# voithru/voice-activity-detection

Hardware: AMD Instinct MI355X
Metric: audio frames/sec (whole node) (higher is better)
Workload: dtype f32 (bf16x6 split operands, f32 accumulate)

## Files before the change

### voice_activity_detection_amd/csrc/savad.hip

```cpp
#include "savad_kernels.h"
#include "savad_kernels_bf16.h"
#include "savad_attn_pw_bf16.h"
#include "savad_packed_bf16.h"
#include "savad_kernels_f32s.h"
#include "savad_generic.h"
#include <type_traits>
#include "savad_logmel.h"
#include "savad_frontend.h"
#include "savad_ingest.h"
#include "savad_post.h"

#include <math.h>
#include <stdarg.h>
#include <stdio.h>
#include <string.h>

#include <map>
#include <mutex>
#include <string>
#include <vector>

#include "../../include/savad.h"

#define SAVAD_EXPORT extern "C" __attribute__((visibility("default")))
// ... 27 lines not shown
constexpr int MAX_EVENTS = 64;

}

struct savad_model {
    savad_config cfg;
    bool generic = false;
    std::vector<Param> params;
    float* d_raw = nullptr;
    float* d_packed = nullptr;
    size_t raw_floats = 0, packed_floats = 0;
    bool dirty = true;
    float* d_pe = nullptr;
    int pe_len = 0;
    std::vector<float> h_pe;
    int splits = 0;
    int row_mode = 0;
    bool batch_invariant = false;
    int precision = 0;
    char* d_frag3 = nullptr;
    size_t frag3_bytes = 0;
    bool frag3_dirty = true;
    bool lds_attrs3_set = false;
    size_t f3_win = 0;
    unsigned* d_sat = nullptr;
    char* d_frag = nullptr;
    size_t frag_bytes = 0;
    bool frag_dirty = true;
    bool lds_attrs_set = false;
    int n_cu = 256;
    size_t f_win = 0;
    struct LayerFrag {
        size_t wqkv, wo, w1, w2;
    };
    std::vector<LayerFrag> lf;
    std::vector<LayerFrag> lf3;
    int prof_capacity = 0, prof_used = 0, prof_nk = 0, prof_skip = 0;
    std::vector<hipEvent_t> events;
    std::vector<const char*> knames;

    size_t r_win, r_bin, r_lnf_w, r_lnf_b, r_wc, r_bc;
    struct LayerRaw {
        size_t wq, bq, wk, bk, wv, bv, wo, bo, ln1w, ln1b, w1, b1, w2, b2, ln2w, ln2b;
    };
    std::vector<LayerRaw> lr;
    struct LayerPacked {
        size_t wqkv, bqkv, w1, b1;
        size_t frag;
    };
    std::vector<LayerPacked> lp;
    size_t p_wc, p_bc;
    size_t p_bias = 0;
    int FP = 0;
    size_t p_win_pad = 0;
};

namespace {

using namespace savad;

size_t add_param(savad_model* m, const std::string& key, size_t numel) {
    const size_t off = m->raw_floats;
    m->params.push_back(Param{key, numel, off, false});
    m->raw_floats += (numel + 3) & ~size_t(3);
    return off;
}

int choose_splits(const savad_model* m, int B, int T) {
    if (T <= 32) return 1;
    const int NT = (T + 31) / 32, QB = NT;
    if (m->splits > 0) return m->splits < NT ? m->splits : NT;
    auto cost = [&](int S) {
        const long wgs = (long)B * ((QB + 3) / 4) * S;
        return (double)((wgs + 255) / 256) * ((NT + S - 1) / S + 1.5);
    };
    const double cost1 = cost(1);
    double best = cost1;
    int bestS = 1;
    for (int S = 2; S <= 8 && S <= NT; ++S) {
        const double cs = cost(S);
// ... 238 lines not shown
#define SAVAD_F32S_PACKED_MIN_BLOCKS 0
#endif
bool packed_f32s_applies(const savad_model* m, int B, int T) {
    if (T > 32 || m->cfg.num_layers > fs::PACKED_F32S_MAX_LAYERS) return false;
    const long nblk = ((long)B + 32 / T - 1) / (32 / T);
    return m->row_mode >= 4 || (m->row_mode == 0 && nblk >= SAVAD_F32S_PACKED_MIN_BLOCKS);
}
#ifndef SAVAD_F32S_MIN_BLOCKS_PER_CU
#define SAVAD_F32S_MIN_BLOCKS_PER_CU 1
#endif
bool f32s_uses_exact_fp32(const savad_model* m, int B, int T) {
    if (m->row_mode != 0) return false;
    if (T <= 32) return !packed_f32s_applies(m, B, T);
    return (long)B * ((T + 31) / 32) <= (long)SAVAD_F32S_MIN_BLOCKS_PER_CU * m->n_cu;
}
int pack_frags3(savad_model* m, hipStream_t st, const float* W, int N, int K, size_t off) {
    const size_t total = (size_t)N * K;
    const int grid = (int)((total + 255) / 256 < 1024 ? (total + 255) / 256 : 1024);
    hipLaunchKernelGGL(fs::pack_weight_frags3_kernel, dim3(grid), dim3(256), 0, st, W, N, K, reinterpret_cast<__bf16*>(m->d_frag3 + off));
    HIP_TRY(hipGetLastError());
    return SAVAD_OK;
}

int prepare_frags3(savad_model* m, hipStream_t st) {
    if (!m->frag3_dirty) return SAVAD_OK;
    const int L = m->cfg.num_layers;
    int rc;
    if ((rc = pack_frags3(m, st, win_fp32(m), D, m->FP, m->f3_win))) return rc;
    for (int l = 0; l < L; ++l) {
        if ((rc = pack_frags3(m, st, m->d_packed + m->lp[l].wqkv, 3 * D, D, m->lf3[l].wqkv))) return rc;
        if ((rc = pack_frags3(m, st, m->d_raw + m->lr[l].wo, D, D, m->lf3[l].wo))) return rc;
        if ((rc = pack_frags3(m, st, m->d_packed + m->lp[l].w1, DFF, D, m->lf3[l].w1))) return rc;
        if ((rc = pack_frags3(m, st, m->d_raw + m->lr[l].w2, D, DFF, m->lf3[l].w2))) return rc;
    }
    m->frag3_dirty = false;
    return SAVAD_OK;
}

template <typename KernelT>
int allow_lds(KernelT kernel, int bytes) {
    HIP_TRY(hipFuncSetAttribute(reinterpret_cast<const void*>(kernel), hipFuncAttributeMaxDynamicSharedMemorySize, bytes));
    return SAVAD_OK;
}

struct Prof {
    savad_model* m;
    hipStream_t st;
    hipEvent_t* ev;
    int n;
    Prof(savad_model* mm, hipStream_t s) : m(mm), st(s), ev(nullptr), n(0) {
        if (m->prof_capacity > 0 && m->prof_skip > 0) {
            --m->prof_skip;
        } else if (m->prof_capacity > 0 && m->prof_used < m->prof_capacity) {
            ev = m->events.data() + (size_t)m->prof_used * MAX_EVENTS;
            m->knames.clear();
            hipEventRecord(ev[0], st);
        }
    }
    void mark(const char* name) {
        if (!ev || n + 1 >= MAX_EVENTS) return;
        ++n;
        hipEventRecord(ev[n], st);
        m->knames.push_back(name);
    }
    void done() {
        if (!ev) return;
// ... 181 lines not shown
    const int F = cfg->feature_size, L = cfg->num_layers;
    m->r_win = add_param(m, "input_layer.0.weight", (size_t)D * F);
    m->r_bin = add_param(m, "input_layer.0.bias", D);
    m->lr.resize(L);
    m->lp.resize(L);
    for (int l = 0; l < L; ++l) {
        const std::string p = "encoder.layers." + std::to_string(l) + ".";
        auto& r = m->lr[l];
        r.wq = add_param(m, p + "self_attention.query_projection.weight", (size_t)D * D);
        r.bq = add_param(m, p + "self_attention.query_projection.bias", D);
        r.wk = add_param(m, p + "self_attention.key_projection.weight", (size_t)D * D);
        r.bk = add_param(m, p + "self_attention.key_projection.bias", D);
        r.wv = add_param(m, p + "self_attention.value_projection.weight", (size_t)D * D);
        r.bv = add_param(m, p + "self_attention.value_projection.bias", D);
        r.wo = add_param(m, p + "self_attention.final_projection.weight", (size_t)D * D);
        r.bo = add_param(m, p + "self_attention.final_projection.bias", D);
        r.ln1w = add_param(m, p + "self_attention_sublayer.layer_norm.weight", D);
        r.ln1b = add_param(m, p + "self_attention_sublayer.layer_norm.bias", D);
        r.w1 = add_param(m, p + "feed_forward.feed_forward.0.weight", (size_t)DFF * D);
        r.b1 = add_param(m, p + "feed_forward.feed_forward.0.bias", DFF);
        r.w2 = add_param(m, p + "feed_forward.feed_forward.3.weight", (size_t)D * DFF);
        r.b2 = add_param(m, p + "feed_forward.feed_forward.3.bias", D);
        r.ln2w = add_param(m, p + "feed_forward_sublayer.layer_norm.weight", D);
        r.ln2b = add_param(m, p + "feed_forward_sublayer.layer_norm.bias", D);
        auto& q = m->lp[l];
        q.wqkv = m->packed_floats;
        m->packed_floats += (size_t)3 * D * D;
        q.bqkv = m->packed_floats;
        m->packed_floats += 3 * D;
        q.w1 = m->packed_floats;
        m->packed_floats += (size_t)DFF * D;
        q.b1 = m->packed_floats;
        m->packed_floats += DFF;
        q.frag = m->packed_floats;
        m->packed_floats += FRAG_LAYER;
    }
    m->r_lnf_w = add_param(m, "encoder.layer_norm.weight", D);
    m->r_lnf_b = add_param(m, "encoder.layer_norm.bias", D);
    m->r_wc = add_param(m, "classifier.weight", 2 * D);
    m->r_bc = add_param(m, "classifier.bias", 2);
    m->p_bias = m->packed_floats;
    m->packed_floats += (size_t)L * LBIAS;
    m->p_wc = m->packed_floats;
    m->packed_floats += 2 * D;
    m->p_bc = m->packed_floats;
    m->packed_floats += 4;
    m->FP = (F + 15) / 16 * 16;
    m->p_win_pad = m->packed_floats;
    m->packed_floats += (size_t)D * m->FP;
    m->lf.resize(L);
    m->f_win = 0;
    m->frag_bytes = (size_t)D * ((F + 15) / 16 * 16) * 2;
    for (int l = 0; l < L; ++l) {
        auto& fl = m->lf[l];
        fl.wqkv = m->frag_bytes;
        m->frag_bytes += (size_t)3 * D * D * 2;
        fl.wo = m->frag_bytes;
        m->frag_bytes += (size_t)D * D * 2;
        fl.w1 = m->frag_bytes;
        m->frag_bytes += (size_t)DFF * D * 2;
        fl.w2 = m->frag_bytes;
        m->frag_bytes += (size_t)D * DFF * 2;
    }
    m->lf3.resize(L);
    m->f3_win = 0;
    m->frag3_bytes = (size_t)D * ((F + 15) / 16 * 16) * 6;
    for (int l = 0; l < L; ++l) {
        auto& fl = m->lf3[l];
        fl.wqkv = m->frag3_bytes;
        m->frag3_bytes += (size_t)3 * D * D * 6;
        fl.wo = m->frag3_bytes;
        m->frag3_bytes += (size_t)D * D * 6;
        fl.w1 = m->frag3_bytes;
        m->frag3_bytes += (size_t)DFF * D * 6;
        fl.w2 = m->frag3_bytes;
        m->frag3_bytes += (size_t)D * DFF * 6;
    }
    hipError_t e = hipMalloc(&m->d_raw, sizeof(float) * m->raw_floats);
    if (e == hipSuccess) e = hipMalloc(&m->d_frag, m->frag_bytes);
    if (e == hipSuccess) e = hipMalloc(&m->d_frag3, m->frag3_bytes);
    if (e == hipSuccess) e = hipMalloc(&m->d_sat, sizeof(unsigned));
    if (e == hipSuccess) e = hipMemset(m->d_sat, 0, sizeof(unsigned));
    if (e == hipSuccess) e = hipMalloc(&m->d_packed, sizeof(float) * m->packed_floats);
    if (e != hipSuccess) {
        if (m->d_raw) hipFree(m->d_raw);
        delete m;
        return fail(SAVAD_E_HIP, "hipMalloc(weights): %s", hipGetErrorString(e));
    }
    *out = m;
    return SAVAD_OK;
}

SAVAD_EXPORT void savad_destroy(savad_handle m) {
    if (!m) return;
    for (hipEvent_t e : m->events) hipEventDestroy(e);
    if (m->d_raw) hipFree(m->d_raw);
    if (m->d_packed) hipFree(m->d_packed);
    if (m->d_frag) hipFree(m->d_frag);
    if (m->d_frag3) hipFree(m->d_frag3);
    if (m->d_sat) hipFree(m->d_sat);
    if (m->d_pe) hipFree(m->d_pe);
    delete m;
}

SAVAD_EXPORT int savad_num_params(savad_handle m) { return m ? (int)m->params.size() : 0; }
SAVAD_EXPORT const char* savad_param_key(savad_handle m, int i) {
    return (m && i >= 0 && i < (int)m->params.size()) ? m->params[i].key.c_str() : nullptr;
}
SAVAD_EXPORT size_t savad_param_numel(savad_handle m, int i) {
// ... 389 lines not shown
    if ((rc = prepare_weights(m, st))) return rc;
    if ((rc = prepare_frags3(m, st))) return rc;
    if ((rc = ensure_pe(m, T, st))) return rc;
    if ((rc = prepare_f32s_launch(m))) return rc;
    char* W = (char*)workspace;
    float* hb = (float*)(W + bp.h);
    const int L = m->cfg.num_layers;
    int F = m->cfg.feature_size;
    if (m->FP != F) {
        float* xp = (float*)(W + bp.xpad);
        const size_t rows = (size_t)B * T;
        const int grid = (int)((rows * m->FP + 255) / 256 < 4096 ? (rows * m->FP + 255) / 256 : 4096);
        hipLaunchKernelGGL(pad_rows_kernel<float>, dim3(grid), dim3(256), 0, st, x, rows, F, m->FP, xp);
        x = xp;
        F = m->FP;
    }
    if (xbs_in > 0 && (m->FP != m->cfg.feature_size || T <= 32)) return fail(SAVAD_E_UNSUPPORTED, "strided input: no kernel takes the stride for this shape");
    const long xbs = xbs_in > 0 ? xbs_in : (long)T * F;
    const float c = (float)(1.4426950408889634 / sqrt((double)D));
    const float* R = m->d_raw;
    const float* P = m->d_packed;
    const char* Fr = m->d_frag3;
    Prof prof(m, st);
    if (packed_f32s_applies(m, B, T)) {
        WindowOffsets none;
        none.w = 0;
        launch_packed_forward_f32s(m, st, x, B, T, F, out, none, 0);
        prof.mark("packed_forward_f32s");
        prof.done();
        HIP_TRY(hipGetLastError());
        return SAVAD_OK;
    }
    char* sets[2][3] = {{W + bp.q, W + bp.k, W + bp.vt}, {W + bp.q2, W + bp.k2, W + bp.vt2}};
    hipLaunchKernelGGL(fs::input_qkv_kernel_f32s, dim3(bp.nblk_pad / 4), dim3(256), fs::NRING3 * fs::SLOT_BYTES + 3 * D * 4, st, x, xbs, B, T, F,
                       bp.nblk, Fr + m->f3_win, R + m->r_bin, m->d_pe, Fr + m->lf3[0].wqkv, P + m->lp[0].bqkv, hb, sets[0][0], sets[0][1],
                       sets[0][2], c);
    prof.mark("input_qkv_f32s");
    const bool packed = T <= 32;
    const int QB = (T + 31) / 32, NG = (QB + 3) / 4;
    const dim3 grid(packed ? bp.nblk_pad / 4 : 8 * (((long)B * NG + 7) / 8));
    for (int l = 0; l < L; ++l) {
        const auto& r = m->lr[l];
        const auto& p = m->lp[l];
        const auto& f = m->lf3[l];
        const bool last = l + 1 == L;
        char** cur = sets[l & 1];
        char** nxt = sets[(l + 1) & 1];
        fs::RowArgs3 A;
        A.B = B;
        A.T = T;
        A.nblk = bp.nblk;
        A.hbuf = hb;
        A.wo_frag = Fr + f.wo;
        A.bo = R + r.bo;
        A.w1_frag = Fr + f.w1;
        A.b1 = P + p.b1;
        A.w2_frag = Fr + f.w2;
        A.b2 = R + r.b2;
        A.wn_frag = last ? nullptr : Fr + m->lf3[l + 1].wqkv;
        A.wc = last ? P + m->p_wc : nullptr;
        A.bn = last ? P + m->p_bc : P + m->lp[l + 1].bqkv;
        A.qf = nxt[0];
        A.kf = nxt[1];
        A.vtf = nxt[2];
        A.out = out;
        A.qscale = c;
        if (packed) {
            if (last) hipLaunchKernelGGL((fs::attention_row_kernel_f32s<true, true>), grid, dim3(256), fs::ROW_LDS_BYTES, st, cur[0], cur[1], cur[2], NG, A);
            else hipLaunchKernelGGL((fs::attention_row_kernel_f32s<false, true>), grid, dim3(256), fs::ROW_LDS_BYTES, st, cur[0], cur[1], cur[2], NG, A);
        } else {
            if (last) hipLaunchKernelGGL((fs::attention_row_kernel_f32s<true, false>), grid, dim3(256), fs::ROW_LDS_BYTES, st, cur[0], cur[1], cur[2], NG, A);
            else hipLaunchKernelGGL((fs::attention_row_kernel_f32s<false, false>), grid, dim3(256), fs::ROW_LDS_BYTES, st, cur[0], cur[1], cur[2], NG, A);
        }
        prof.mark(last ? "attention_row_last_f32s" : "attention_row_f32s");
    }
    prof.done();
    HIP_TRY(hipGetLastError());
    return SAVAD_OK;
}

}

namespace {
void launch_packed_forward(savad_model* m, hipStream_t st, const float* x, int B, int T, int F, float* out, const WindowOffsets& wo,
                           int win_base) {
    const int L = m->cfg.num_layers;
    const float* R = m->d_raw;
    const float* P = m->d_packed;
    const float c = (float)(1.4426950408889634 / sqrt((double)D));
    const int G = 32 / T, nblk = (B + G - 1) / G;
    PackedModel pm;
    for (int l = 0; l < L; ++l) pm.layer[l] = PackedLayer{P + m->lp[l].frag};
    for (int l = L; l < PACKED_MAX_LAYERS; ++l) pm.layer[l] = pm.layer[0];
    pm.bias = P + m->p_bias;
// ... 1207 lines not shown
```

### voice_activity_detection_amd/csrc/savad_kernels_f32s.h

```cpp
#pragma once
#include "savad_kernels_bf16.h"
#include <type_traits>

namespace savad {
#ifdef SAVAD_TIMING
__device__ long long g_savad_wg[1024][4];
#endif
namespace fs {

using bf::bf16x8;
using bf::u32x4;
using bf::ldfrag;
using bf::stfrag;
using bf::FRAG_BYTES;
using bf::slot_row;
using bf::AttnState;
using bf::attn_state_init;
using bf::online_softmax_shifted;

constexpr int TFRAG_BYTES = 3 * FRAG_BYTES;
constexpr int BLK3_BYTES = 8 * TFRAG_BYTES;
constexpr int SLOT_BYTES = 2 * BLK3_BYTES;
constexpr int NRING3 = 3;
constexpr int HBLK_BYTES = 32 * D * 4;
// ... 52 lines not shown
__device__ __forceinline__ Tri zero_tri() {
    const bf16x8 z = __builtin_bit_cast(bf16x8, u32x4{0u, 0u, 0u, 0u});
    return Tri{z, z, z};
}

#define SAVAD_MF(a, b, c) __builtin_amdgcn_mfma_f32_32x32x16_bf16((a), (b), (c), 0, 0, 0)
template <bool SWAP>
__device__ __forceinline__ void mfma6x2_lo(f32x16& acc0, f32x16& acc1, const Tri& a0, const Tri& a1, const Tri& b) {
#define SAVAD_MF2(pa, pb)                                                           \
    acc0 = SWAP ? SAVAD_MF(b.pb, a0.pa, acc0) : SAVAD_MF(a0.pa, b.pb, acc0);        \
    acc1 = SWAP ? SAVAD_MF(b.pb, a1.pa, acc1) : SAVAD_MF(a1.pa, b.pb, acc1);
    SAVAD_MF2(h, l) SAVAD_MF2(l, h) SAVAD_MF2(m, m)
}
template <bool SWAP>
__device__ __forceinline__ void mfma6x2_hi(f32x16& acc0, f32x16& acc1, const Tri& a0, const Tri& a1, const Tri& b) {
    SAVAD_MF2(h, m) SAVAD_MF2(m, h) SAVAD_MF2(h, h)
#undef SAVAD_MF2
}
template <bool SWAP>
__device__ __forceinline__ void mfma6x2(f32x16& acc0, f32x16& acc1, const Tri& a0, const Tri& a1, const Tri& b) {
    mfma6x2_lo<SWAP>(acc0, acc1, a0, a1, b);
    mfma6x2_hi<SWAP>(acc0, acc1, a0, a1, b);
}

__device__ __forceinline__ void load_hblock32(f32x16 (&x)[4], const float* hb, int lane) {
#pragma unroll
    for (int nb = 0; nb < 4; ++nb)
#pragma unroll
        for (int g = 0; g < 4; ++g) {
            const f32x4 t = ld4(hb + ((nb * 4 + g) * 64 + lane) * 4);
#pragma unroll
            for (int s = 0; s < 4; ++s) x[nb][4 * g + s] += t[s];
        }
}
__device__ __forceinline__ void store_hblock32(float* hb, const f32x16 (&x)[4], int lane) {
#pragma unroll
    for (int nb = 0; nb < 4; ++nb)
#pragma unroll
        for (int g = 0; g < 4; ++g) {
            f32x4 t;
#pragma unroll
            for (int s = 0; s < 4; ++s) t[s] = x[nb][4 * g + s];
            st4(hb + ((nb * 4 + g) * 64 + lane) * 4, t);
        }
}

#ifndef SAVAD_PIECE_FENCE
#define SAVAD_PIECE_FENCE 0x6
#endif
struct DmaJob {
    const char* src;
    unsigned ldsb;
};
struct Ring3 {
    static constexpr int PER = 12;
    char* base;
    int w, lane;
    unsigned voff[3];

    __device__ __forceinline__ Ring3(char* smem, int w_, int lane_) : base(smem), w(w_), lane(lane_) {
#pragma unroll
        for (int g = 0; g < 3; ++g) voff[g] = (unsigned)lane_ * 16u + 4096u * g;
    }
    __device__ __forceinline__ char* slot(int t) const { return base + (t % NRING3) * SLOT_BYTES; }
    __device__ __forceinline__ DmaJob job(int t, const char* seg0, const char* seg1) const {
        const unsigned slot0 = __builtin_amdgcn_readfirstlane((unsigned)(size_t)slot(t));
// ... 54 lines not shown
        const Tri w1_{__builtin_bit_cast(bf16x8, f[(ks) & 1][3]), __builtin_bit_cast(bf16x8, f[(ks) & 1][4]),                  \
                      __builtin_bit_cast(bf16x8, f[(ks) & 1][5])};                                                            \
        mfma6x2_lo<SWAP>(acc0, acc1, w0_, w1_, xp[ks]);                                                                       \
        if constexpr (DMA && (P1) >= 0) ring.template piece<((P1) >= 0 ? (P1) : 0)>(job);                                     \
        mfma6x2_hi<SWAP>(acc0, acc1, w0_, w1_, xp[ks]);                                                                       \
        if constexpr (DMA) ring.template piece<P0>(job);                                                                      \
    }
    SAVAD_G_LD6(0);
    SAVAD_G_STEP(0, 1, 0) SAVAD_G_STEP(1, 2, -1) SAVAD_G_STEP(2, 4, 3) SAVAD_G_STEP(3, 5, -1)
    SAVAD_G_STEP(4, 7, 6) SAVAD_G_STEP(5, 8, -1) SAVAD_G_STEP(6, 10, 9) SAVAD_G_STEP(7, 11, -1)
#undef SAVAD_G_STEP
#undef SAVAD_G_LD6
#undef SAVAD_G_LD
}

__global__ void pack_weight_frags3_kernel(const float* __restrict__ W, int N, int K, __bf16* __restrict__ out) {
    const int KS = K / 16;
    const size_t total = (size_t)(N / 32) * KS * 64 * 8;
    for (size_t i = (size_t)blockIdx.x * blockDim.x + threadIdx.x; i < total; i += (size_t)gridDim.x * blockDim.x) {
        const int e = (int)(i & 7);
        const int lane = (int)((i >> 3) & 63);
        const size_t f = i >> 9;
        const int ks = (int)(f % KS);
        const int nblk = (int)(f / KS);
        const int n = lane & 31, h = lane >> 5;
        const int k = 32 * (ks >> 1) + 16 * (ks & 1) + 8 * (e >> 2) + 4 * h + (e & 3);
        __bf16 ph, pm, pl;
        split1(W[(size_t)(32 * nblk + n) * K + k], ph, pm, pl);
        const size_t o = f * 3 * 512 + (size_t)lane * 8 + e;
        out[o] = ph;
        out[o + 512] = pm;
        out[o + 1024] = pl;
    }
}

template <int S, bool DMA>
__device__ __forceinline__ void qkv_slot(const char* slot, const Tri (&xp)[8], const float* lbq, char* __restrict__ qf, char* __restrict__ kf,
                                         char* __restrict__ vtf, int blk, const Ring3& ring, const DmaJob& job, float qscale, bool live) {
    const int lane = ring.lane, n = lane & 31, h = lane >> 5;
    constexpr int rb = S >> 1, nb0 = 2 * (S & 1);
    f32x16 acc[2];
    if constexpr (rb < 2) {
#pragma unroll
        for (int i = 0; i < 2; ++i) acc[i] = bias_block(lbq + D * rb + 32 * (nb0 + i), h);
        gemm_slot<false, DMA>(acc[0], acc[1], slot, xp, ring, job);
    } else {
#pragma unroll
        for (int i = 0; i < 2; ++i) {
            const float bv = lbq[2 * D + 32 * (nb0 + i) + n];
#pragma unroll
            for (int r = 0; r < 16; ++r) acc[i][r] = bv;
        }
        gemm_slot<true, DMA>(acc[0], acc[1], slot, xp, ring, job);
    }
    if constexpr (rb == 0) {
        acc[0] *= qscale;
        acc[1] *= qscale;
    }
    if (!live) return;
    char* dst = rb == 0 ? qf : (rb == 1 ? kf : vtf);
#pragma unroll
    for (int i = 0; i < 2; ++i)
#pragma unroll
        for (int j = 0; j < 2; ++j)
            sttri(dst + (size_t)blk * BLK3_BYTES + (2 * (nb0 + i) + j) * TFRAG_BYTES + lane * 16, split_half(acc[i], j));
}
// ... 243 lines not shown
        sb = SAVAD_MF(k.h, qp[ks].m, sb);
        sa = SAVAD_MF(k.m, qp[ks].h, sa);
        sb = SAVAD_MF(k.h, qp[ks].h, sb);
    }
    f32x16 sc = sa + sb;
    mask(sc);
    online_softmax_shifted(sc, st, true);
    const Tri p0 = split_half(sc, 0), p1 = split_half(sc, 1);
#pragma unroll
    for (int nbd = 0; nbd < 4; nbd += 2) {
        mfma6x2<false>(st.O[nbd], st.O[nbd + 1], ldtri(vtblk + ((nbd * 2 + 0) * TFRAG_BYTES) + lane * 16),
                       ldtri(vtblk + (((nbd + 1) * 2 + 0) * TFRAG_BYTES) + lane * 16), p0);
        mfma6x2<false>(st.O[nbd], st.O[nbd + 1], ldtri(vtblk + ((nbd * 2 + 1) * TFRAG_BYTES) + lane * 16),
                       ldtri(vtblk + (((nbd + 1) * 2 + 1) * TFRAG_BYTES) + lane * 16), p1);
    }
}

struct RowArgs3 {
    int B, T, nblk;
    float* hbuf;
    const char* wo_frag;
    const float* bo;
    const char* w1_frag;
    const float* b1;
    const char* w2_frag;
    const float* b2;
    const char* wn_frag;
    const float* wc;
    const float* bn;
    char *qf, *kf, *vtf;
    float* out;
    float qscale;
};
__device__ __forceinline__ const char* row_seg(const RowArgs3& A, int t, int sgm) {
    if (t < 2) return A.wo_frag + (size_t)(2 * t + sgm) * BLK3_BYTES;
    if (t < 18) {
        const int c = (t - 2) >> 2, r = (t - 2) & 3;
        return r < 2 ? A.w1_frag + (size_t)(4 * c + 2 * r + sgm) * BLK3_BYTES
                     : A.w2_frag + (size_t)((2 * (r - 2) + sgm) * 32 + 8 * c) * TFRAG_BYTES;
    }
    return A.wn_frag + (size_t)(2 * (t - 18) + sgm) * BLK3_BYTES;
}

template <bool LAST>
struct RowBiases {
    BiasPiece pieces[4];
    BiasRegs<4> regs;
    float bc;
    float* lbn;
    __device__ __forceinline__ RowBiases(const RowArgs3& A, char* smem) {
        float* lbo = reinterpret_cast<float*>(smem + NRING3 * SLOT_BYTES);
        float* lb1 = lbo + D;
        float* lb2 = lb1 + DFF;
        lbn = lb2 + D;
        pieces[0] = BiasPiece{lbo, A.bo, D};
        pieces[1] = BiasPiece{lb1, A.b1, DFF};
        pieces[2] = BiasPiece{lb2, A.b2, D};
        pieces[3] = BiasPiece{lbn, LAST ? A.wc : A.bn, LAST ? 2 * D : 3 * D};
        regs = request_bias_pieces(pieces);
        bc = LAST ? A.bn[threadIdx.x & 1] : 0.0f;
    }
    __device__ __forceinline__ void commit() const {
        commit_bias_pieces(pieces, regs);
        if (LAST && threadIdx.x < 2) lbn[2 * D + threadIdx.x] = bc;
    }
};

template <bool LAST, bool PREFETCHED>
__device__ __forceinline__ void row_stage_f32s(const RowArgs3& A, char* smem, Tri (&xp)[8], int blk, bool live, const Ring3& ring, int base) {
    float* lbo = reinterpret_cast<float*>(smem + NRING3 * SLOT_BYTES);
    float* lb1 = lbo + D;
    float* lb2 = lb1 + DFF;
    float* lbn = lb2 + D;
    const int lane = ring.lane, m = lane & 31, h = lane >> 5;
    constexpr int NSLOT = LAST ? 18 : 24;
    auto job = [&](int t) { return ring.job(base + t, row_seg(A, t, 0), row_seg(A, t, 1)); };
    const DmaJob none{nullptr, 0u};
    if (!PREFETCHED) {
        ring.issue_all(job(0));
        ring.issue_all(job(1));
    }
#define SAVAD_ROW_GEMM(T_, acc0, acc1, operand)                                                                               \
    if ((T_) < 8) SAVAD_STAMP(24 + 3 * (T_));                                                                                 \
    ring.acquire<((T_) + 1 < NSLOT) ? 1 : 0>();                                                                               \
    if ((T_) < 8) SAVAD_STAMP(25 + 3 * (T_));                                                                                 \
    gemm_slot<false, ((T_) + 2 < NSLOT)>(acc0, acc1, ring.slot(base + (T_)), operand, ring, (T_) + 2 < NSLOT ? job((T_) + 2) : none); \
    if ((T_) < 8) SAVAD_STAMP(26 + 3 * (T_));
    float* hb = A.hbuf + (size_t)blk * (32 * D);
    ring.acquire<1>();
    f32x16 hres[4];
#pragma unroll
    for (int nb = 0; nb < 4; ++nb) hres[nb] = zero16();
    if (live) load_hblock32(hres, hb, lane);
    f32x16 h1[4];
#pragma unroll
    for (int nb = 0; nb < 4; ++nb) h1[nb] = bias_block(lbo + 32 * nb, h);
    gemm_slot<false, true>(h1[0], h1[1], ring.slot(base), xp, ring, job(2));
    SAVAD_ROW_GEMM(1, h1[2], h1[3], xp)
#pragma unroll
    for (int nb = 0; nb < 4; ++nb) h1[nb] += hres[nb];
    SAVAD_STAMP(5);
    f32x4 xg[16];
    layernorm_regs(h1, xg);
    split_row(xg, xp);
    SAVAD_STAMP(6);
    f32x16(&o)[4] = h1;
#pragma unroll
    for (int nb = 0; nb < 4; ++nb) o[nb] += bias_block(lb2 + 32 * nb, h);
#define SAVAD_ROW_FFN(ch)                                                                                                     \
    {                                                                                                                         \
        f32x16 a[4];                                                                                                          \
        _Pragma("unroll") for (int nbl = 0; nbl < 4; ++nbl) a[nbl] = bias_block(lb1 + 128 * (ch) + 32 * nbl, h);              \
        SAVAD_ROW_GEMM(2 + 4 * (ch), a[0], a[1], xp)                                                                          \
        SAVAD_ROW_GEMM(3 + 4 * (ch), a[2], a[3], xp)                                                                          \
        if ((ch) == 0) SAVAD_STAMP(20);                                                                                       \
        Tri ap[8];                                                                                                            \
        _Pragma("unroll") for (int nbl = 0; nbl < 4; ++nbl) {                                                                 \
            _Pragma("unroll") for (int r = 0; r < 16; ++r) a[nbl][r] = fmaxf(a[nbl][r], 0.0f);                                \
            ap[2 * nbl] = split_half(a[nbl], 0);                                                                              \
            ap[2 * nbl + 1] = split_half(a[nbl], 1);                                                                          \
        }                                                                                                                     \
        if ((ch) == 0) SAVAD_STAMP(21);                                                                                       \
        SAVAD_ROW_GEMM(4 + 4 * (ch), o[0], o[1], ap)                                                                          \
        SAVAD_ROW_GEMM(5 + 4 * (ch), o[2], o[3], ap)                                                                          \
        SAVAD_STAMP(7 + (ch));                                                                                                \
    }
    SAVAD_ROW_FFN(0) SAVAD_ROW_FFN(1) SAVAD_ROW_FFN(2) SAVAD_ROW_FFN(3)
#undef SAVAD_ROW_FFN
#undef SAVAD_ROW_GEMM
    if (!LAST && live) store_hblock32(hb, o, lane);
    layernorm_regs(o, xg);
    if constexpr (!LAST) {
        split_row(xg, xp);
        SAVAD_STAMP(11);
#define SAVAD_ROW_QKV(S_)                                                                                                     \
    ring.acquire<(18 + (S_) + 1 < NSLOT) ? 1 : 0>();                                                                          \
    qkv_slot<S_, (18 + (S_) + 2 < NSLOT)>(ring.slot(base + 18 + (S_)), xp, lbn, A.qf, A.kf, A.vtf, blk, ring,                 \
                                          18 + (S_) + 2 < NSLOT ? job(18 + (S_) + 2) : none, A.qscale, live);                 \
    SAVAD_STAMP(12 + (S_));
        SAVAD_ROW_QKV(0) SAVAD_ROW_QKV(1) SAVAD_ROW_QKV(2) SAVAD_ROW_QKV(3) SAVAD_ROW_QKV(4) SAVAD_ROW_QKV(5)
#undef SAVAD_ROW_QKV
    } else {
        float z0 = 0.0f, z1 = 0.0f;
#pragma unroll
        for (int G = 0; G < 16; ++G) {
            const f32x4 c0 = ld4(lbn + 8 * G + 4 * h), c1 = ld4(lbn + D + 8 * G + 4 * h);
#pragma unroll
            for (int e = 0; e < 4; ++e) {
                z0 = __builtin_fmaf(xg[G][e], c0[e], z0);
                z1 = __builtin_fmaf(xg[G][e], c1[e], z1);
            }
        }
        z0 = half_sum(z0) + lbn[2 * D];
        z1 = half_sum(z1) + lbn[2 * D + 1];
        const float mx = fmaxf(z0, z1);
        const float lse = mx + logf(expf(z0 - mx) + expf(z1 - mx));
        size_t row;
        int t_frame;
        const bool valid = live && (blk < A.nblk) && slot_row(A.B, A.T, blk, m, row, t_frame);
        if (h == 0 && valid) *reinterpret_cast<f32x2*>(A.out + row * 2) = f32x2{z0 - lse, z1 - lse};
    }
}

template <bool LAST, bool PACKED>
__global__ __launch_bounds__(256, 1) void attention_row_kernel_f32s(const char* __restrict__ qf, const char* __restrict__ kf,
                                                                    const char* __restrict__ vtf, int NG, RowArgs3 A) {
    extern __shared__ __attribute__((aligned(16))) char smem[];
    const int B = A.B, T = A.T;
    const int lane = threadIdx.x & 63, m = lane & 31, h = lane >> 5;
    const int w = __builtin_amdgcn_readfirstlane(threadIdx.x >> 6);
    const Ring3 ring(smem, w, lane);
    AttnState st;
    attn_state_init(st);
    Tri qp[8];
    int blk_q, base = 0;
    bool active, qvalid;
    SAVAD_STAMP(0);
#ifdef SAVAD_TIMING
    if (threadIdx.x == 0 && blockIdx.x < 1024) {
        g_savad_wg[blockIdx.x][0] = __builtin_readcyclecounter();
        g_savad_wg[blockIdx.x][2] = __builtin_amdgcn_s_memrealtime();
    }
#endif
    const RowBiases<LAST> biases(A, smem);
    if constexpr (PACKED) {
        biases.commit();
        blk_q = blockIdx.x * 4 + w;
        active = blk_q < A.nblk;
        const int G = 32 / T;
        qvalid = active && (m < G * T) && (blk_q * G + m / T < B);
        if (active) {
#pragma unroll
            for (int ks = 0; ks < 8; ++ks) qp[ks] = ldtri(qf + (size_t)blk_q * BLK3_BYTES + ks * TFRAG_BYTES + lane * 16);
            bool keyok[16];
#pragma unroll
            for (int r = 0; r < 16; ++r) {
                const int jk = 8 * (r >> 2) + 4 * h + (r & 3);
                keyok[r] = (jk < G * T) && (jk / T == m / T) && (blk_q * G + jk / T < B);
            }
            auto mask = [&](f32x16& sc) {
#pragma unroll
                for (int r = 0; r < 16; ++r) sc[r] = keyok[r] ? sc[r] : NEG_BIG;
            };
            attn_tile3_global(st, qp, kf + (size_t)blk_q * BLK3_BYTES, vtf + (size_t)blk_q * BLK3_BYTES, mask, lane);
        }
    } else {
        const int QB = (T + 31) / 32;
        int b, g;
        if (!xcd_balanced_map(B, NG, b, g)) return;
        const int qb0 = (g * QB) / NG, qb1 = ((g + 1) * QB) / NG;
        const int qb = qb0 + w;
        active = qb < qb1;
        blk_q = b * QB + (active ? qb : qb0);
        qvalid = active && 32 * qb + m < T;
        base = QB;
        auto job = [&](int u) {
            if (u < QB) {
                const size_t kb = (size_t)b * QB;
                const int uv = u < 0 ? 0 : u, uk = u + 1 < QB ? u + 1 : QB - 1;
                return ring.job(u + 3, vtf + (kb + uv) * BLK3_BYTES, kf + (kb + uk) * BLK3_BYTES);
            }
            return ring.job(u, row_seg(A, u - QB, 0), row_seg(A, u - QB, 1));
        };
        ring.issue_all(job(-1));
#pragma unroll
        for (int ks = 0; ks < 8; ++ks) qp[ks] = ldtri(qf + (size_t)blk_q * BLK3_BYTES + ks * TFRAG_BYTES + lane * 16);
        ring.issue_all(job(0));
        ring.issue_all(job(1));
        biases.commit();
        const int lim = T - 32 * (QB - 1) - 4 * h;
        auto no_mask = [](f32x16&) {};
        auto tail_mask = [&](f32x16& sc) {
            if (32 * QB > T) {
                asm volatile("" ::: "memory");
#pragma unroll
                for (int r = 0; r < 16; ++r) sc[r] = (8 * (r >> 2) + (r & 3) < lim) ? sc[r] : NEG_BIG;
            }
        };
        ring.acquire<2>();
        SAVAD_STAMP(1);
        if (active) {
            f32x16 sc = qk_tile3(st, qp, ring.slot(2) + BLK3_BYTES, lane);
            settle_reference(sc, st, true);
            SAVAD_STAMP(2);
#pragma unroll 1
            for (int jt = 0; jt + 2 < QB; ++jt) {
                ring.acquire<1>();
                attn_step3<true, true>(st, qp, sc, ring.slot(jt), no_mask, ring, job(jt + 2));
            }
            ring.acquire<1>();
            attn_step3<true, true>(st, qp, sc, ring.slot(QB - 2), tail_mask, ring, job(QB));
            ring.acquire<1>();
            attn_step3<false, true>(st, qp, sc, ring.slot(QB - 1), no_mask, ring, job(QB + 1));
            SAVAD_STAMP(3);
        } else {
#pragma unroll 1
            for (int jt = 0; jt < QB; ++jt) {
                ring.acquire<1>();
                ring.issue_all(job(jt + 2));
            }
        }
    }
    Tri xp[8];
    {
        const float inv = qvalid ? 1.0f / half_sum(st.l_run) : 0.0f;
#pragma unroll
        for (int nbd = 0; nbd < 4; ++nbd) {
#pragma unroll
            for (int r = 0; r < 16; ++r) st.O[nbd][r] = qvalid ? st.O[nbd][r] * inv : 0.0f;
            xp[2 * nbd] = split_half(st.O[nbd], 0);
            xp[2 * nbd + 1] = split_half(st.O[nbd], 1);
        }
    }
    SAVAD_STAMP(4);
    row_stage_f32s<LAST, !PACKED>(A, smem, xp, blk_q, active, ring, base);
    SAVAD_STAMP(18);
#ifdef SAVAD_TIMING
    if (threadIdx.x == 0 && blockIdx.x < 1024) {
        g_savad_wg[blockIdx.x][1] = __builtin_readcyclecounter();
        g_savad_wg[blockIdx.x][3] = __builtin_amdgcn_s_memrealtime();
    }
#endif
}

constexpr int PACKED_F32S_MAX_LAYERS = 3;
struct PackedF32sLayer {
    const char *wqkv, *wo, *w1, *w2;
};
struct PackedF32sModel {
    PackedF32sLayer layer[PACKED_F32S_MAX_LAYERS];
    const char* win;
    const float* bin;
    const float* pe;
    const float* bias;
    const float *wc, *bc;
    int L;
};
inline constexpr int packed_f32s_lds_bytes(int L) { return NRING3 * SLOT_BYTES + (L * LBIAS + 2 * D + 4) * 4; }
__device__ __forceinline__ const char* packed_seg(const PackedF32sLayer& Lw, int i, int sgm) {
    if (i < 6) return Lw.wqkv + (size_t)(2 * i + sgm) * BLK3_BYTES;
    if (i < 8) return Lw.wo + (size_t)(2 * (i - 6) + sgm) * BLK3_BYTES;
    const int c = (i - 8) >> 2, r = (i - 8) & 3;
    return r < 2 ? Lw.w1 + (size_t)(4 * c + 2 * r + sgm) * BLK3_BYTES : Lw.w2 + (size_t)((2 * (r - 2) + sgm) * 32 + 8 * c) * TFRAG_BYTES;
}

__global__ __launch_bounds__(256, 1) void packed_forward_kernel_f32s(const float* __restrict__ x, int B, int T, int F, int nblk,
                                                                     PackedF32sModel M, float qscale, float* __restrict__ out,
                                                                     WindowOffsets wo, int win_base) {
// ... 543 lines not shown
```

Before: 80.94 million.

## Fold output projection into V weights for the unpacked attention path

Precomputes Wvo = Wo·Wv and the matching folded bias in double precision, packing a separate QKV fragment set whose V projection already includes the attention output projection. In the non-packed (T>32) path the row stage then skips the two Wo GEMM slots and adds the attention output directly to the residual. It also issues the residual h-block loads early, during the last attention step, so they overlap compute. The trade-offs are extra weight memory and a different rounding path for the folded product. The ring schedule is also re-indexed, which risks off-by-slot mistakes.

```diff
diff --git a/voice_activity_detection_amd/csrc/savad.hip b/voice_activity_detection_amd/csrc/savad.hip
--- a/voice_activity_detection_amd/csrc/savad.hip
+++ b/voice_activity_detection_amd/csrc/savad.hip
@@ -83,6 +83,7 @@
     size_t f_win = 0;
     struct LayerFrag {
         size_t wqkv, wo, w1, w2;
+        size_t wqkv_vo = 0;
     };
     std::vector<LayerFrag> lf;
     std::vector<LayerFrag> lf3;
@@ -97,6 +98,7 @@
     std::vector<LayerRaw> lr;
     struct LayerPacked {
         size_t wqkv, bqkv, w1, b1;
+        size_t wvo, bqkv_vo;
         size_t frag;
     };
     std::vector<LayerPacked> lp;
@@ -401,6 +403,12 @@
         if ((rc = pack_frags3(m, st, m->d_raw + m->lr[l].wo, D, D, m->lf3[l].wo))) return rc;
         if ((rc = pack_frags3(m, st, m->d_packed + m->lp[l].w1, DFF, D, m->lf3[l].w1))) return rc;
         if ((rc = pack_frags3(m, st, m->d_raw + m->lr[l].w2, D, DFF, m->lf3[l].w2))) return rc;
+        const auto& p = m->lp[l];
+        hipLaunchKernelGGL(fs::fold_vo_kernel, dim3(D), dim3(D), 0, st, m->d_raw + m->lr[l].wo, m->d_packed + p.wqkv + (size_t)2 * D * D,
+                           m->d_packed + p.bqkv, m->d_packed + p.wvo, m->d_packed + p.bqkv_vo);
+        HIP_TRY(hipGetLastError());
+        if ((rc = pack_frags3(m, st, m->d_packed + p.wqkv, 2 * D, D, m->lf3[l].wqkv_vo))) return rc;
+        if ((rc = pack_frags3(m, st, m->d_packed + p.wvo, D, D, m->lf3[l].wqkv_vo + (size_t)2 * D * D * 6))) return rc;
     }
     m->frag3_dirty = false;
     return SAVAD_OK;
@@ -648,6 +656,10 @@
         m->packed_floats += (size_t)DFF * D;
         q.b1 = m->packed_floats;
         m->packed_floats += DFF;
+        q.wvo = m->packed_floats;
+        m->packed_floats += (size_t)D * D;
+        q.bqkv_vo = m->packed_floats;
+        m->packed_floats += 3 * D;
         q.frag = m->packed_floats;
         m->packed_floats += FRAG_LAYER;
     }
@@ -691,6 +703,8 @@
         m->frag3_bytes += (size_t)DFF * D * 6;
         fl.w2 = m->frag3_bytes;
         m->frag3_bytes += (size_t)D * DFF * 6;
+        fl.wqkv_vo = m->frag3_bytes;
+        m->frag3_bytes += (size_t)3 * D * D * 6;
     }
     hipError_t e = hipMalloc(&m->d_raw, sizeof(float) * m->raw_floats);
     if (e == hipSuccess) e = hipMalloc(&m->d_frag, m->frag_bytes);
@@ -1146,11 +1160,12 @@
         return SAVAD_OK;
     }
     char* sets[2][3] = {{W + bp.q, W + bp.k, W + bp.vt}, {W + bp.q2, W + bp.k2, W + bp.vt2}};
+    const bool packed = T <= 32;
+    auto wqkv3 = [&](int l) { return Fr + (packed ? m->lf3[l].wqkv : m->lf3[l].wqkv_vo); };
+    auto bqkv3 = [&](int l) { return P + (packed ? m->lp[l].bqkv : m->lp[l].bqkv_vo); };
     hipLaunchKernelGGL(fs::input_qkv_kernel_f32s, dim3(bp.nblk_pad / 4), dim3(256), fs::NRING3 * fs::SLOT_BYTES + 3 * D * 4, st, x, xbs, B, T, F,
-                       bp.nblk, Fr + m->f3_win, R + m->r_bin, m->d_pe, Fr + m->lf3[0].wqkv, P + m->lp[0].bqkv, hb, sets[0][0], sets[0][1],
-                       sets[0][2], c);
+                       bp.nblk, Fr + m->f3_win, R + m->r_bin, m->d_pe, wqkv3(0), bqkv3(0), hb, sets[0][0], sets[0][1], sets[0][2], c);
     prof.mark("input_qkv_f32s");
-    const bool packed = T <= 32;
     const int QB = (T + 31) / 32, NG = (QB + 3) / 4;
     const dim3 grid(packed ? bp.nblk_pad / 4 : 8 * (((long)B * NG + 7) / 8));
     for (int l = 0; l < L; ++l) {
@@ -1171,9 +1186,9 @@
         A.b1 = P + p.b1;
         A.w2_frag = Fr + f.w2;
         A.b2 = R + r.b2;
-        A.wn_frag = last ? nullptr : Fr + m->lf3[l + 1].wqkv;
+        A.wn_frag = last ? nullptr : wqkv3(l + 1);
         A.wc = last ? P + m->p_wc : nullptr;
-        A.bn = last ? P + m->p_bc : P + m->lp[l + 1].bqkv;
+        A.bn = last ? P + m->p_bc : bqkv3(l + 1);
         A.qf = nxt[0];
         A.kf = nxt[1];
         A.vtf = nxt[2];
diff --git a/voice_activity_detection_amd/csrc/savad_kernels_f32s.h b/voice_activity_detection_amd/csrc/savad_kernels_f32s.h
--- a/voice_activity_detection_amd/csrc/savad_kernels_f32s.h
+++ b/voice_activity_detection_amd/csrc/savad_kernels_f32s.h
@@ -108,6 +108,18 @@
 #pragma unroll
             for (int s = 0; s < 4; ++s) x[nb][4 * g + s] += t[s];
         }
+}
+__device__ __forceinline__ void request_hblock32(f32x4 (&hr)[16], const float* hb , int lane) {
+#define SAVAD_H_LD(i)                                                                                                          \
+    asm volatile("global_load_dwordx4 %0, %1, %2 offset:%3" : "+v"(hr[i]) : "v"((unsigned)lane * 16u + 4096u * ((i) / 4)), "s"(hb), \
+                 "n"(((i) % 4) * 1024) : "memory")
+    SAVAD_H_LD(0); SAVAD_H_LD(1); SAVAD_H_LD(2); SAVAD_H_LD(3); SAVAD_H_LD(4); SAVAD_H_LD(5); SAVAD_H_LD(6); SAVAD_H_LD(7);
+    SAVAD_H_LD(8); SAVAD_H_LD(9); SAVAD_H_LD(10); SAVAD_H_LD(11); SAVAD_H_LD(12); SAVAD_H_LD(13); SAVAD_H_LD(14); SAVAD_H_LD(15);
+#undef SAVAD_H_LD
+}
+__device__ __forceinline__ void landed_hblock32(f32x4 (&hr)[16]) {
+    asm volatile("" : "+v"(hr[0]), "+v"(hr[1]), "+v"(hr[2]), "+v"(hr[3]), "+v"(hr[4]), "+v"(hr[5]), "+v"(hr[6]), "+v"(hr[7]), "+v"(hr[8]),
+                 "+v"(hr[9]), "+v"(hr[10]), "+v"(hr[11]), "+v"(hr[12]), "+v"(hr[13]), "+v"(hr[14]), "+v"(hr[15]));
 }
 __device__ __forceinline__ void store_hblock32(float* hb, const f32x16 (&x)[4], int lane) {
 #pragma unroll
@@ -228,6 +240,20 @@
         out[o + 512] = pm;
         out[o + 1024] = pl;
     }
+}
+
+__global__ void fold_vo_kernel(const float* __restrict__ Wo, const float* __restrict__ Wv, const float* __restrict__ bqkv,
+                               float* __restrict__ Wvo, float* __restrict__ bqkv_vo) {
+    const int n = blockIdx.x, k = threadIdx.x;
+    double acc = 0.0, accb = 0.0;
+    for (int j = 0; j < D; ++j) {
+        const double w = (double)Wo[(size_t)n * D + j];
+        acc += w * (double)Wv[(size_t)j * D + k];
+        accb += w * (double)bqkv[2 * D + j];
+    }
+    Wvo[(size_t)n * D + k] = (float)acc;
+    if (k == 0) bqkv_vo[2 * D + n] = (float)accb;
+    if (n < 2) bqkv_vo[n * D + k] = bqkv[n * D + k];
 }
 
 template <int S, bool DMA>
@@ -537,14 +563,17 @@
     float* out;
     float qscale;
 };
-__device__ __forceinline__ const char* row_seg(const RowArgs3& A, int t, int sgm) {
-    if (t < 2) return A.wo_frag + (size_t)(2 * t + sgm) * BLK3_BYTES;
-    if (t < 18) {
-        const int c = (t - 2) >> 2, r = (t - 2) & 3;
+__device__ __forceinline__ const char* row_seg(const RowArgs3& A, int t, int sgm, bool folded) {
+    if (!folded) {
+        if (t < 2) return A.wo_frag + (size_t)(2 * t + sgm) * BLK3_BYTES;
+        t -= 2;
+    }
+    if (t < 16) {
+        const int c = t >> 2, r = t & 3;
         return r < 2 ? A.w1_frag + (size_t)(4 * c + 2 * r + sgm) * BLK3_BYTES
                      : A.w2_frag + (size_t)((2 * (r - 2) + sgm) * 32 + 8 * c) * TFRAG_BYTES;
     }
-    return A.wn_frag + (size_t)(2 * (t - 18) + sgm) * BLK3_BYTES;
+    return A.wn_frag + (size_t)(2 * (t - 16) + sgm) * BLK3_BYTES;
 }
 
 template <bool LAST>
@@ -571,39 +600,50 @@
     }
 };
 
-template <bool LAST, bool PREFETCHED>
-__device__ __forceinline__ void row_stage_f32s(const RowArgs3& A, char* smem, Tri (&xp)[8], int blk, bool live, const Ring3& ring, int base) {
+template <bool LAST, bool FOLDED>
+__device__ __forceinline__ void row_stage_f32s(const RowArgs3& A, char* smem, Tri (&xp)[8], const f32x16 (&hc)[4], f32x4 (&hr)[16], int blk,
+                                               bool live, const Ring3& ring, int base) {
     float* lbo = reinterpret_cast<float*>(smem + NRING3 * SLOT_BYTES);
     float* lb1 = lbo + D;
     float* lb2 = lb1 + DFF;
     float* lbn = lb2 + D;
     const int lane = ring.lane, m = lane & 31, h = lane >> 5;
-    constexpr int NSLOT = LAST ? 18 : 24;
-    auto job = [&](int t) { return ring.job(base + t, row_seg(A, t, 0), row_seg(A, t, 1)); };
+    constexpr int OFF = FOLDED ? 0 : 2;
+    constexpr int NSLOT = OFF + (LAST ? 16 : 22);
+    auto job = [&](int t) { return ring.job(base + t, row_seg(A, t, 0, FOLDED), row_seg(A, t, 1, FOLDED)); };
     const DmaJob none{nullptr, 0u};
-    if (!PREFETCHED) {
-        ring.issue_all(job(0));
-        ring.issue_all(job(1));
-    }
 #define SAVAD_ROW_GEMM(T_, acc0, acc1, operand)                                                                               \
     if ((T_) < 8) SAVAD_STAMP(24 + 3 * (T_));                                                                                 \
-    ring.acquire<((T_) + 1 < NSLOT) ? 1 : 0>();                                                                               \
+    if constexpr (!(FOLDED && (T_) == 0)) ring.acquire<((T_) + 1 < NSLOT) ? 1 : 0>();    \
     if ((T_) < 8) SAVAD_STAMP(25 + 3 * (T_));                                                                                 \
     gemm_slot<false, ((T_) + 2 < NSLOT)>(acc0, acc1, ring.slot(base + (T_)), operand, ring, (T_) + 2 < NSLOT ? job((T_) + 2) : none); \
     if ((T_) < 8) SAVAD_STAMP(26 + 3 * (T_));
     float* hb = A.hbuf + (size_t)blk * (32 * D);
-    ring.acquire<1>();
-    f32x16 hres[4];
-#pragma unroll
-    for (int nb = 0; nb < 4; ++nb) hres[nb] = zero16();
-    if (live) load_hblock32(hres, hb, lane);
     f32x16 h1[4];
-#pragma unroll
-    for (int nb = 0; nb < 4; ++nb) h1[nb] = bias_block(lbo + 32 * nb, h);
-    gemm_slot<false, true>(h1[0], h1[1], ring.slot(base), xp, ring, job(2));
-    SAVAD_ROW_GEMM(1, h1[2], h1[3], xp)
-#pragma unroll
-    for (int nb = 0; nb < 4; ++nb) h1[nb] += hres[nb];
+    if constexpr (FOLDED) {
+        ring.acquire<1>();
+        landed_hblock32(hr);
+#pragma unroll
+        for (int nb = 0; nb < 4; ++nb) {
+            h1[nb] = bias_block(lbo + 32 * nb, h) + hc[nb];
+#pragma unroll
+            for (int r = 0; r < 16; ++r) h1[nb][r] += hr[4 * nb + (r >> 2)][r & 3];
+        }
+    } else {
+        ring.issue_all(job(0));
+        ring.issue_all(job(1));
+        ring.acquire<1>();
+        f32x16 hres[4];
+#pragma unroll
+        for (int nb = 0; nb < 4; ++nb) hres[nb] = zero16();
+        if (live) load_hblock32(hres, hb, lane);
+#pragma unroll
+        for (int nb = 0; nb < 4; ++nb) h1[nb] = bias_block(lbo + 32 * nb, h);
+        gemm_slot<false, true>(h1[0], h1[1], ring.slot(base), xp, ring, job(2));
+        SAVAD_ROW_GEMM(1, h1[2], h1[3], xp)
+#pragma unroll
+        for (int nb = 0; nb < 4; ++nb) h1[nb] += hres[nb];
+    }
     SAVAD_STAMP(5);
     f32x4 xg[16];
     layernorm_regs(h1, xg);
@@ -616,8 +656,8 @@
     {                                                                                                                         \
         f32x16 a[4];                                                                                                          \
         _Pragma("unroll") for (int nbl = 0; nbl < 4; ++nbl) a[nbl] = bias_block(lb1 + 128 * (ch) + 32 * nbl, h);              \
-        SAVAD_ROW_GEMM(2 + 4 * (ch), a[0], a[1], xp)                                                                          \
-        SAVAD_ROW_GEMM(3 + 4 * (ch), a[2], a[3], xp)                                                                          \
+        SAVAD_ROW_GEMM(OFF + 4 * (ch), a[0], a[1], xp)                                                                        \
+        SAVAD_ROW_GEMM(OFF + 1 + 4 * (ch), a[2], a[3], xp)                                                                          \
         if ((ch) == 0) SAVAD_STAMP(20);                                                                                       \
         Tri ap[8];                                                                                                            \
         _Pragma("unroll") for (int nbl = 0; nbl < 4; ++nbl) {                                                                 \
@@ -626,8 +666,8 @@
             ap[2 * nbl + 1] = split_half(a[nbl], 1);                                                                          \
         }                                                                                                                     \
         if ((ch) == 0) SAVAD_STAMP(21);                                                                                       \
-        SAVAD_ROW_GEMM(4 + 4 * (ch), o[0], o[1], ap)                                                                          \
-        SAVAD_ROW_GEMM(5 + 4 * (ch), o[2], o[3], ap)                                                                          \
+        SAVAD_ROW_GEMM(OFF + 2 + 4 * (ch), o[0], o[1], ap)                                                                    \
+        SAVAD_ROW_GEMM(OFF + 3 + 4 * (ch), o[2], o[3], ap)                                                                          \
         SAVAD_STAMP(7 + (ch));                                                                                                \
     }
     SAVAD_ROW_FFN(0) SAVAD_ROW_FFN(1) SAVAD_ROW_FFN(2) SAVAD_ROW_FFN(3)
@@ -639,9 +679,9 @@
         split_row(xg, xp);
         SAVAD_STAMP(11);
 #define SAVAD_ROW_QKV(S_)                                                                                                     \
-    ring.acquire<(18 + (S_) + 1 < NSLOT) ? 1 : 0>();                                                                          \
-    qkv_slot<S_, (18 + (S_) + 2 < NSLOT)>(ring.slot(base + 18 + (S_)), xp, lbn, A.qf, A.kf, A.vtf, blk, ring,                 \
-                                          18 + (S_) + 2 < NSLOT ? job(18 + (S_) + 2) : none, A.qscale, live);                 \
+    ring.acquire<(OFF + 16 + (S_) + 1 < NSLOT) ? 1 : 0>();                                                                    \
+    qkv_slot<S_, (OFF + 16 + (S_) + 2 < NSLOT)>(ring.slot(base + OFF + 16 + (S_)), xp, lbn, A.qf, A.kf, A.vtf, blk, ring,     \
+                                                OFF + 16 + (S_) + 2 < NSLOT ? job(OFF + 16 + (S_) + 2) : none, A.qscale, live); \
     SAVAD_STAMP(12 + (S_));
         SAVAD_ROW_QKV(0) SAVAD_ROW_QKV(1) SAVAD_ROW_QKV(2) SAVAD_ROW_QKV(3) SAVAD_ROW_QKV(4) SAVAD_ROW_QKV(5)
 #undef SAVAD_ROW_QKV
@@ -680,6 +720,9 @@
     Tri qp[8];
     int blk_q, base = 0;
     bool active, qvalid;
+    f32x4 hr[16];
+#pragma unroll
+    for (int i = 0; i < 16; ++i) hr[i] = f32x4{0.f, 0.f, 0.f, 0.f};
     SAVAD_STAMP(0);
 #ifdef SAVAD_TIMING
     if (threadIdx.x == 0 && blockIdx.x < 1024) {
@@ -725,7 +768,7 @@
                 const int uv = u < 0 ? 0 : u, uk = u + 1 < QB ? u + 1 : QB - 1;
                 return ring.job(u + 3, vtf + (kb + uv) * BLK3_BYTES, kf + (kb + uk) * BLK3_BYTES);
             }
-            return ring.job(u, row_seg(A, u - QB, 0), row_seg(A, u - QB, 1));
+            return ring.job(u, row_seg(A, u - QB, 0, true), row_seg(A, u - QB, 1, true));
         };
         ring.issue_all(job(-1));
 #pragma unroll
@@ -756,6 +799,7 @@
             ring.acquire<1>();
             attn_step3<true, true>(st, qp, sc, ring.slot(QB - 2), tail_mask, ring, job(QB));
             ring.acquire<1>();
+            request_hblock32(hr, A.hbuf + (size_t)blk_q * (32 * D), lane);
             attn_step3<false, true>(st, qp, sc, ring.slot(QB - 1), no_mask, ring, job(QB + 1));
             SAVAD_STAMP(3);
         } else {
@@ -773,12 +817,14 @@
         for (int nbd = 0; nbd < 4; ++nbd) {
 #pragma unroll
             for (int r = 0; r < 16; ++r) st.O[nbd][r] = qvalid ? st.O[nbd][r] * inv : 0.0f;
-            xp[2 * nbd] = split_half(st.O[nbd], 0);
-            xp[2 * nbd + 1] = split_half(st.O[nbd], 1);
+            if constexpr (PACKED) {
+                xp[2 * nbd] = split_half(st.O[nbd], 0);
+                xp[2 * nbd + 1] = split_half(st.O[nbd], 1);
+            }
         }
     }
     SAVAD_STAMP(4);
-    row_stage_f32s<LAST, !PACKED>(A, smem, xp, blk_q, active, ring, base);
+    row_stage_f32s<LAST, !PACKED>(A, smem, xp, st.O, hr, blk_q, active, ring, base);
     SAVAD_STAMP(18);
 #ifdef SAVAD_TIMING
     if (threadIdx.x == 0 && blockIdx.x < 1024) {
```

Result: faster. 83.76 million (median of 6 runs) (+3.5%).
